# martin-velas/SLAM_plus_plus

Measured on AMD Instinct MI355X. Metric: Lambda solve GFLOP/s (algorithmic factor+solve flops / wall-clock), 100k-pose SE(3), higher is better.
Workload: dtype f64; 1 GPU; C3: synthetic 100000-pose SE(3) chain + loop closures, 6x6 blocks, 201998 upper blocks, n=600000; numeric factor + 2 substitutions per step (symbolic analysis cached, inputs resident in HBM); parallelism=1 GPU

## Files before the change

### slam_plus_plus_amd/csrc/panel_kernel.hip

```cpp
#include <hip/hip_runtime.h>
#include "sparse_kernels.h"

namespace slampp {

#include "sparse_device.inl"

template <int D, int BATCH>
__device__ __forceinline__ void panel_update_block(const TUpdSlot &sl, bool b_valid, const TUpdEnt *__restrict__ ents,
	const double *__restrict__ A, double *L, const double *__restrict__ b, double *w, int n_sub_wave, int n_waves, int lane,
	double *s_ops , double *s_yv , double *s_part )
{
	enum { DD = D * D };
	const TLaneMap mm = lane_map(lane, D, D);
	const bool b_diag = sl.kind != 0;
	const bool b_y = b_diag && lane >= Y_LANE0 && lane < Y_LANE0 + D;
	const int yq = b_y? lane - Y_LANE0 : mm.q;
	double init = 0;
	if(b_valid && n_sub_wave == 0)
		init = b_y? b[sl.cs_src + yq] : (mm.b_act? lambda_element(A, sl.asrc, mm.r, mm.q, D, D, false) : 0.0);
	double sum = 0;
	const TUpdEnt *p_ent = ents + sl.e0;
	const int ne = b_valid? sl.ne : 0;
	for(int e0 = n_sub_wave * BATCH; e0 < ne; e0 += n_waves * BATCH) {
		const int n_here = min(int(BATCH), ne - e0);
// ... 397 lines not shown
			const double init = b_y? s_w[ci * D + yq] : (mm.b_act? s_L[col.slot0 * DD + lane] : 0.0);
			double sum = 0;
			for(int e = 0; e < col.inr; ++ e) {
				const uint32_t en = s_irow[col.ir0 + e];
				sum += row_product_image<D>(s_L + int(en & 0xffff) * DD, s_w + int(en >> 16) * D, mm.r, yq, b_y);
			}
			TColDesc cd;
			cd.linv_off = col.linv_off;
			cd.cs_new = col.cs_new;
			const double acc = init - sum;
			finish_diagonal_fixed<D>(cd, acc, acc, lane, b_y? 0 : mm.r, b_y? 0 : mm.q, mm.b_act, L, Linv, w, s_slot[col.slot0].loff,
				p_flag, s_linv + (ci - ci0) * 64, s_L + col.slot0 * DD, s_w + ci * D);
		}
		__syncthreads();
		PANEL_TICK();
		int n_before = 0;
		for(int ci = ci0; ci < ci1; ++ ci) {
			const int n_slot0 = s_col[ci].slot0, n_nb = s_col[ci].nb;
			for(int kb = 1 + ((wave - n_before) % W + W) % W; kb < n_nb; kb += W) {
				const int n_slot = n_slot0 + kb;
				const TPanelSlot sd = s_slot[n_slot];
				const double init = mm.b_act? s_L[n_slot * DD + lane] : 0.0;
				double sum = 0;
				for(int e = 0; e < sd.inp; ++ e) {
					const uint32_t en = s_ipair[sd.ip0 + e];
					sum += pair_product_image<D>(s_L + int(en & 0xffff) * DD, s_L + int(en >> 16) * DD, mm.r, mm.q);
				}
				finish_offdiagonal<D>(init - sum, lane, mm.r, mm.q, mm.b_act, D, L, sd.loff, s_tile, s_linv + (ci - ci0) * 64, s_L + n_slot * DD);
			}
			n_before += n_nb - 1;
		}
		__syncthreads();
		PANEL_TICK();
		ci0 = ci1;
	}
	panel_hand_up<D>(s_out, n_out, 0, n_out, wave, W, lane, mm, b_y, yq, s_L, s_w, H);
	PANEL_TICK();
}

bool launch_factor_panel(int n_dim, bool b_fused, bool b_rows, const TPanelLaunch &r_cfg, const longlong2 *pkg, const int64_t *pkg_off, const int64_t *out_off,
	int n_tasks, const TUpdSlot *upd_slots, int n_upd_slots, const TUpdEnt *upd_ents, const double *A, const double *b, double *L, double *Linv, double *w,
	double *H, int *p_flag, hipStream_t stream, long long *p_timing, const TBatch &t_batch)
{
	if(!b_fused)
		n_upd_slots = 0;
	const int W = r_cfg.n_waves, n_groups = W / std::min(W, int(PANEL_UPD_W));
	const int n_grid = n_tasks + (n_upd_slots + n_groups - 1) / n_groups;
	if(n_grid <= 0)
		return true;
	const size_t n_lds_bytes = size_t(panel_lds(n_dim, b_fused, r_cfg).TOTAL) * sizeof(double);
	if(n_lds_bytes > PANEL_LDS_BUDGET)
		return false;
#define LAUNCH_PANEL_INSTANCE(D, WW, F, RW) do { \
		static bool b_attribute_set = false; \
		if(!b_attribute_set) { \
			(void)hipFuncSetAttribute(reinterpret_cast<const void*>(&factor_panel_kernel<D, WW, F, RW>), hipFuncAttributeMaxDynamicSharedMemorySize, 160 * 1024); \
			b_attribute_set = true; \
		} \
		hipLaunchKernelGGL((factor_panel_kernel<D, WW, F, RW>), dim3(n_grid, t_batch.n), dim3(64 * WW), n_lds_bytes, stream, pkg, pkg_off, out_off, n_tasks, r_cfg, \
			upd_slots, n_upd_slots, upd_ents, A, b, L, Linv, w, H, p_flag, p_timing, t_batch); } while(0)
#define LAUNCH_PANEL_F(D, WW, F) do { if(b_rows) LAUNCH_PANEL_INSTANCE(D, WW, F, true); else LAUNCH_PANEL_INSTANCE(D, WW, F, false); } while(0)
#define LAUNCH_PANEL(D) do { \
		if(W == 2) { if(b_fused) LAUNCH_PANEL_F(D, 2, true); else LAUNCH_PANEL_F(D, 2, false); } \
		else if(W == 4) { if(b_fused) LAUNCH_PANEL_F(D, 4, true); else LAUNCH_PANEL_F(D, 4, false); } \
		else { if(b_fused) LAUNCH_PANEL_F(D, 8, true); else LAUNCH_PANEL_F(D, 8, false); } } while(0)
	switch(n_dim) {
	case 3:
		LAUNCH_PANEL(3);
		return true;
	case 6:
		LAUNCH_PANEL(6);
		return true;
	case 7:
		LAUNCH_PANEL(7);
		return true;
	default:
		return false;
	}
#undef LAUNCH_PANEL
#undef LAUNCH_PANEL_F
#undef LAUNCH_PANEL_INSTANCE
}

template <int D>
__global__ void __launch_bounds__(64 * PANEL_UPD_W)
panel_update_kernel(const TUpdSlot *__restrict__ slots, const TUpdEnt *__restrict__ ents, const double *__restrict__ A, double *L,
	const double *__restrict__ b, double *w, TBatch t_batch)
{	{ const int64_t n_member = blockIdx.y; A += n_member * t_batch.a; L += n_member * t_batch.l; b += n_member * t_batch.b; w += n_member * t_batch.w; }

	enum { W = PANEL_UPD_W, DD = D * D, BATCH = 8 };
	__shared__ double s_ops[W][2 * BATCH * DD];
	__shared__ double s_yv[W][BATCH * 8];
	__shared__ double s_part[W][64];
	const int wave = threadIdx.x >> 6, lane = threadIdx.x & 63;
	const TUpdSlot sl = slots[blockIdx.x];
	panel_update_block<D, BATCH>(sl, true, ents, A, L, b, w, wave, W, lane, s_ops[wave], s_yv[wave], s_part[0]);
}

void launch_panel_update(int n_dim, const TUpdSlot *slots, int n_slots, const TUpdEnt *ents, const double *A, double *L,
	const double *b, double *w, hipStream_t stream, const TBatch &t_batch)
{
	if(n_slots <= 0)
		return;
	if(n_dim == 3)
		hipLaunchKernelGGL((panel_update_kernel<3>), dim3(n_slots, t_batch.n), dim3(64 * PANEL_UPD_W), 0, stream, slots, ents, A, L, b, w, t_batch);
	else if(n_dim == 6)
		hipLaunchKernelGGL((panel_update_kernel<6>), dim3(n_slots, t_batch.n), dim3(64 * PANEL_UPD_W), 0, stream, slots, ents, A, L, b, w, t_batch);
	else
		hipLaunchKernelGGL((panel_update_kernel<7>), dim3(n_slots, t_batch.n), dim3(64 * PANEL_UPD_W), 0, stream, slots, ents, A, L, b, w, t_batch);
}

}

#include "preload.h"
SLAMPP_PRELOAD_UNIT(panel_kernel)
```

### slam_plus_plus_amd/csrc/solver.h

```cpp
#pragma once
#include <hip/hip_runtime.h>
#include <chrono>
#include <cstdint>
#include <new>
#include <stdexcept>
#include <string>
#include <vector>
#include <thread>
#include <memory>
#include <mutex>

#include "../../include/slampp_hip.h"
#include "plan.h"
#include <utility>
#include "sparse_kernels.h"
#include "dense_chol.h"

namespace slampp {

struct CDeviceError : public std::runtime_error {
	explicit CDeviceError(const std::string &s) :std::runtime_error(s) {}
};

#define SLAMPP_HIP_CHECK(call) do { hipError_t e_ = (call); if(e_ != hipSuccess) { \
// ... 81 lines not shown
template <class T> using raw_vector = std::vector<T, CNoInitAlloc<T> >;

struct TTrash { virtual ~TTrash() {} };
template <class T> struct TTrashOf : TTrash { T t; explicit TTrashOf(T &r) { t.swap(r); } };
typedef std::vector<std::unique_ptr<TTrash> > CTrashList;
template <class T> inline void Discard_Later(CTrashList &r_trash, T &r_v) { r_trash.emplace_back(new TTrashOf<T>(r_v)); }

struct CKeepDeviceMemory {
	bool b_before;
	CKeepDeviceMemory() :b_before(g_b_keep_device_memory) { g_b_keep_device_memory = true; }
	~CKeepDeviceMemory() { g_b_keep_device_memory = b_before; }
};

struct CSchurState;
struct CDeviceGroup;
struct CSparseInverse;
struct CCovariance;
struct CAssemblyState;

}

struct slampp_hip_assembly {
	slampp_hip_solver *p_solver;
	slampp::CAssemblyState *p_state;
	bool b_stale;
};

struct slampp_hip_solver {
	int n_device;
	hipStream_t stream;
	std::string s_error;
	slampp::PlanOptions opt;
	int n_dense_nb;
	int b_shard_primary;
	int n_shard_rank, n_shard_world;
	int n_marginals_dense;
	int n_assembly_groups = 1 << 20;
	int n_schur_tiles = -1;
	int n_schur_incremental = 0;
	int n_schur_sparse;

	bool b_has_structure, b_analyzed, b_factored;
	uint64_t n_factor_gen = 0, n_schur_cov_gen = 0;
	int n_mode;
	int64_t n_matrix_cut;
	std::vector<int64_t> cumsum, bcol_ptr;
	std::vector<int32_t> brow;
	int64_t n_values, n_scalars;

	bool b_refined = false;
	int64_t n_refined_values = 0;
	std::vector<int64_t> refined_cumsum, refined_bcol_ptr;
	std::vector<int32_t> refined_brow;
	slampp::CDevArray<int64_t> d_refine_map;
	slampp::CDevArray<double> d_refined;
	void Refine_Structure();
	bool b_schur_fallback = false;
	int n_staging_ahead = 0;
	int n_schur_fallback_option = 1;
	slampp::Plan plan;
	int n_bottom_stages;
	slampp::TDevPlan dplan;
	slampp::CDevArray<slampp::TColDesc> d_cols;
	slampp::CDevArray<slampp::TBlkDesc> d_blks;
	slampp::CDevArray<slampp::TRowEnt> d_rents;
	slampp::CDevArray<longlong2> d_pairs;
	slampp::CDevArray<int64_t> d_task_ptr, d_task_pkg;
	slampp::CDevArray<longlong2> d_pkg;
	slampp::CDevArray<long long> d_timing;
	slampp::CDevArray<slampp::TSimtChunk> d_simt_chunks;
	slampp::CDevArray<int32_t> d_simt_prog, d_simt_rest;
	int n_panel = -1;
	int n_panel_rows = -1;
	slampp::CDevArray<longlong2> d_panel_pkg;
	slampp::CDevArray<int64_t> d_panel_off, d_panel_out_off;
	slampp::CDevArray<double> d_handup;
	bool b_any_hand_up = false;
	int n_panel_handup = 1;
	slampp::CDevArray<int32_t> d_panel_rest;
	slampp::CDevArray<slampp::TUpdSlot> d_panel_upd_slots;
	slampp::CDevArray<slampp::TUpdEnt> d_panel_upd_ents;
	std::vector<int32_t> panel_ptr, panel_rest_ptr, panel_upd_ptr;
	std::vector<slampp::TPanelLaunch> panel_cfg;
	std::vector<char> panel_ride;
	slampp::CDevArray<int64_t> d_simt_tab;
	slampp::CDevArray<slampp::TSimtChunk> d_simt_bwd_chunks;
	slampp::CDevArray<int32_t> d_simt_bwd_prog;
	slampp::CDevArray<int64_t> d_simt_bwd_tab;
	std::vector<int32_t> simt_bwd_lds_bytes;
	std::vector<slampp::TSimtChunk> simt_host_bwd_chunks;
	std::vector<int32_t> simt_host_bwd_prog;
	slampp::raw_vector<int64_t> simt_host_bwd_tab;
	bool b_leaf_linv_wanted = false, b_leaf_linv_valid = true;
	slampp::TBatch t_batch = slampp::t_No_Batch();
	slampp::CDevArray<double> d_batch_L, d_batch_Linv, d_batch_w, d_batch_handup;
	slampp::CDevArray<int> d_batch_flag;
	int n_batch_owner_member = -1;
	int *p_host_batch_flag = 0;
	int n_batch_pending = 0;
	int n_simt_backward = -1;
	void Ensure_Leaf_Inverses();
	std::vector<int32_t> simt_chunk_ptr, simt_rest_ptr;
	std::vector<int32_t> simt_lds_bytes;
	int n_simt = -1;
	int n_wide_min_tasks = 8192;
	int n_simt_width = 32;
	int n_simt_stages = 1;
	void Build_Simt();
	void Upload_Simt();
	std::vector<slampp::TSimtChunk> simt_host_chunks;
	std::vector<int32_t> simt_host_prog, simt_host_rest;
	slampp::raw_vector<int64_t> simt_host_tab;
	slampp::CDevArray<slampp::TDenseBlk> d_dense_blks;
	slampp::CDevArray<int64_t> d_dense_blk_loff;
	slampp::CDevArray<double> d_dense, d_dense_invdiag, d_dense_z, d_dense_x;
	slampp::CDevArray<int32_t> d_dense_gaps;
	int n_dense_gaps;
	slampp::CDevArray<uint8_t> d_dense_unit;
	slampp::CDevArray<longlong2> d_dense_dst;
	slampp::CTileSchedule dense_tiles;
	bool b_dense_tiles;
	bool b_dense_clean;
	int n_dense_top_tiles;
	int n_dense_blks, n_dense_cols, n_dense_dim, n_dense_pad;
	slampp::CDevArray<double> d_A, d_rhs, d_L, d_Linv, d_w, d_cov;
	slampp::CSparseInverse *p_sinv = 0;
	bool b_sinv_tried = false;
	slampp::CCovariance *p_cov = 0;
	slampp::CDevArray<double> d_Z;
	slampp::CDevArray<double> d_Zd, d_Zd_work;
	slampp::CDevArray<int64_t> d_diag_zoff;
	slampp::CDevArray<int32_t> d_diag_dim;
	slampp::CDevArray<int64_t> d_diag_out_off;
	slampp::CDevArray<int64_t> d_damp_off;
	bool b_damp_valid = false;
	slampp::CDevArray<int> d_flag;
	int *p_flag_shared = 0;
	int *p_host_flag;

	double *p_pin_values = 0, *p_pin_rhs = 0;
	size_t n_pin_values = 0, n_pin_rhs = 0;
	bool b_pin_values_registered = false, b_pin_rhs_registered = false;
	bool b_pin_values_deferred = false, b_pin_rhs_deferred = false;
	bool b_staging_ever = false;
	std::thread t_staging_registration;
	void Register_Staging_Later();
	void Join_Staging_Registration();
	slampp::CTrashList analysis_trash;
	std::thread t_discard;
	void Join_Discard() { if(t_discard.joinable()) t_discard.join(); }
	std::thread t_bringup;
	std::mutex m_bringup;
	int n_bringup_status = SLAMPP_HIP_OK;
	int n_Join_Bringup()
	{
		std::lock_guard<std::mutex> t_lock(m_bringup);
		if(t_bringup.joinable()) {
			const double t0 = slampp::wall_ms();
			t_bringup.join();
			if(getenv("SLAMPP_HIP_PLAN_TIMING"))
				fprintf(stderr, "[bring-up] waited for %.2f ms\n", slampp::wall_ms() - t0);
		}
		return n_bringup_status;
	}
	void Join_Bringup()
	{
// ... 96 lines not shown
```

### slam_plus_plus_amd/csrc/sparse_enqueue.hip

```cpp
#include <execinfo.h>
#include <signal.h>
#include <unistd.h>
#include <pthread.h>
#include "solver.h"
#include "sparse_inverse.h"

#include <algorithm>
#include <atomic>
#include <chrono>
#include <cstdio>
#include <cstdlib>
#include <cstring>
#include <map>
#include <thread>
#include <mutex>
#include <condition_variable>
#include <functional>
#include <sys/mman.h>

using namespace slampp;

void slampp_hip_solver::Enqueue_Sparse(const double *p_values_dev, double *p_rhs_dev, bool b_factor, bool b_factor_only)
{
	const Plan &P = plan;
// ... 60 lines not shown
				}
			} else if(s == 0 && !panel_ptr.empty() && panel_ptr[1] > panel_ptr[0]) {
				Launch_Panels(s, true);
			} else if(s > 0 && s < n_bottom_stages && dplan.task_pkg)
				launch_factor_wide(dplan, p_values_dev, d_L.p(), d_Linv.p(), p_rhs_dev, d_w.p(), P.stage_ptr[s],
					P.stage_ptr[s + 1] - P.stage_ptr[s], p_flag, stream, t_batch);
			else if(s >= n_bottom_stages && !panel_ptr.empty()) {
				Launch_Panels(s, false);
			} else
			launch_factor_stage(dplan, p_values_dev, d_L.p(), d_Linv.p(), p_rhs_dev, d_w.p(), P.stage_ptr[s],
				P.stage_ptr[s + 1] - P.stage_ptr[s], s < n_bottom_stages, p_flag, stream, t_batch);
			if(s == 0 || (s == n_wide_end - 1 && b_profile >= 2) || s == n_stages - 1)
				Phase_End();
		}
	} else {
		Phase_Begin("forward");
		for(int s = 0; s < n_stages; ++ s) {
			launch_forward_stage(dplan, d_L.p(), d_Linv.p(), p_rhs_dev, d_w.p(), P.stage_ptr[s],
				P.stage_ptr[s + 1] - P.stage_ptr[s], stream);
		}
		Phase_End();
	}
	if(b_factor_only && !n_dense_dim) {
		SLAMPP_HIP_CHECK(hipGetLastError());
		return;
	}
	if(n_dense_dim) {
		const int ld = n_dense_pad;
		if(b_factor) {
			Phase_Begin("dense_assemble");
			if(b_dense_tiles && b_dense_clean)
				tile_zero(dense_tiles, d_dense.p(), ld, stream, d_dense_unit.p());
			else {
				SLAMPP_HIP_CHECK(hipMemsetAsync(d_dense.p(), 0, size_t(ld) * ld * sizeof(double), stream));
				b_dense_clean = b_dense_tiles;
				dense_prepare_padding(d_dense.p(), ld, n_dense_dim, stream);
				dense_prepare_gaps(d_dense.p(), ld, d_dense_gaps.p(), n_dense_gaps, stream);
			}
			launch_dense_assemble(dplan, d_dense_blks.p(), n_dense_blks, p_values_dev, d_L.p(), p_rhs_dev, d_w.p(),
				d_dense.p(), ld, false, stream);
			Phase_End();
			Phase_Begin("dense_chol");
			if(b_dense_tiles)
				tile_cholesky(dense_tiles, d_dense.p(), ld, n_dense_dim, d_dense_invdiag.p(), p_flag, stream);
			else
				dense_cholesky(d_dense.p(), ld, n_dense_dim, d_dense_invdiag.p(), p_flag, stream);
			Phase_End();
			if(b_factor_only) {
				launch_dense_gather_factor(d_dense_blks.p(), d_dense_blk_loff.p(), n_dense_blks, d_dense.p(), ld, d_L.p(), stream);
				SLAMPP_HIP_CHECK(hipGetLastError());
				return;
			}
		} else {
			Phase_Begin("dense_forward");
			launch_dense_assemble(dplan, d_dense_blks.p(), n_dense_blks, 0, d_L.p(), p_rhs_dev, d_w.p(),
				d_dense.p(), ld, true, stream);
			dense_forwardsolve(d_dense.p(), ld, d_dense_invdiag.p(), stream);
			Phase_End();
		}
		Phase_Begin("dense_solve");
		if(b_dense_tiles)
			tile_backsolve(dense_tiles, d_dense.p(), ld, n_dense_dim, d_dense_invdiag.p(), d_dense_z.p(), d_dense_x.p(), stream,
				d_dense_dst.p(), d_w.p(), p_rhs_dev);
		else
		dense_backsolve(d_dense.p(), ld, n_dense_dim, d_dense_invdiag.p(), d_dense_z.p(), d_dense_x.p(), stream,
			d_dense_dst.p(), d_w.p(), p_rhs_dev);
		Phase_End();
	}
	Phase_Begin("backward");
	for(int s = n_stages; s > 0; -- s) {
		if(b_simt_bwd && s < int(simt_chunk_ptr.size())) {
			const int n_chunks = simt_chunk_ptr[s] - simt_chunk_ptr[s - 1], n_rest = simt_rest_ptr[s] - simt_rest_ptr[s - 1];
			launch_backward_simt(d_simt_bwd_chunks.p() + simt_chunk_ptr[s - 1], n_chunks, n_simt_width, simt_bwd_lds_bytes[s - 1],
				d_simt_bwd_prog.p(), d_simt_bwd_tab.p(), P.max_dim, d_L.p(), d_w.p(), p_rhs_dev, stream, t_batch);
			if(n_rest > 0) {
				TDevPlan t_rest = dplan;
				t_rest.task_map = d_simt_rest.p();
				launch_backward_stage(t_rest, d_L.p(), d_Linv.p(), d_w.p(), p_rhs_dev, simt_rest_ptr[s - 1], n_rest, stream, t_batch);
			}
			continue;
		}
		if(s < int(simt_chunk_ptr.size()))
			Ensure_Leaf_Inverses();
		launch_backward_stage(dplan, d_L.p(), d_Linv.p(), d_w.p(), p_rhs_dev, P.stage_ptr[s - 1],
			P.stage_ptr[s] - P.stage_ptr[s - 1], stream, t_batch);
	}
	Phase_End();
	SLAMPP_HIP_CHECK(hipGetLastError());
}
```

### slam_plus_plus_amd/csrc/sparse_kernels.h

```cpp
#pragma once
#include <hip/hip_runtime.h>
#include <stdint.h>
#include "plan.h"

namespace slampp {

struct TBatch {
	int n;
	int64_t a, l, linv, b, w, h;
};
inline TBatch t_No_Batch() { TBatch t = {1, 0, 0, 0, 0, 0, 0}; return t; }



struct TColDesc {
	int64_t k0;
	int32_t nb, dj;
	int64_t linv_off;
	int64_t cs_new;
	int64_t cs_src;
	int64_t r0;
	int32_t nr;
	int32_t np;
	int64_t p0;
};

struct TBlkDesc {
	int64_t loff;
	int64_t asrc;
	int64_t p0;
	uint32_t np_di;
	int32_t xcs;
};

struct TRowEnt {
	int64_t off;
	int32_t ycs;
	int32_t dc;
};

struct TDenseBlk {
	int64_t asrc;
	int64_t p0;
	int64_t dst;
	int64_t r0;
	int32_t np, nr;
	int32_t di, dj;
	int64_t cs_src;
	int32_t pos;
	int32_t pad;
};

struct TDenseCol {
	int64_t cs_new, cs_src;
	int32_t pos, dj;
};

enum { PANEL_W = 8, PANEL_COLS = 8, PANEL_UNITS = 1024, PANEL_UPD_W = 4 };
struct TPanelHead {
	int32_t n_cols, n_slots, n_units, n_int_rows;
	int32_t ext_ptr[12];
};
struct TPanelOut {
	int32_t op0, onp;
	int64_t dst;
};
struct TPanelCol {
	int64_t linv_off, cs_new, cs_src;
	int32_t slot0, nb;
	int32_t ir0, inr;
	int32_t sub, pad;
};
struct TPanelSlot {
	int64_t loff, asrc;
	int32_t ip0, inp;
	int64_t pad;
};
struct TPanelExt {
	int64_t a_off, b_off;
	int32_t ycs;
	uint16_t slot, kind;
	int32_t col;
	int32_t pad;
};
struct TUpdSlot {
	int64_t loff, asrc;
	int64_t e0;
	int32_t ne, kind;
	int64_t cs_src, cs_new;
	int64_t pad[2];
};
struct TUpdEnt {
	int64_t a_off;
	int64_t b_off;
};
inline int panel_slot_cap(int n_dim) { return (n_dim == 6)? 96 : (n_dim == 7)? 72 : 256; }

struct TPanelLaunch {
	int32_t n_waves, n_cap_units, n_cap_blk, n_cap_cols, n_cap_lvl;
	int32_t n_cap_out;
	int32_t b_from_lambda;
};
enum { PANEL_UPD_BATCH = 8 };
inline __host__ __device__ constexpr int panel_fresh_batch(int n_waves) { return (n_waves == 4)? 8 : 4; }
struct TPanelLds {
	int IMAGE, VEC, LINV, TILE, OPS, YV, OUT, TOTAL;
};
enum { PANEL_LDS_BUDGET = 156 * 1024 };
inline __host__ __device__ TPanelLds panel_lds(int D, bool b_fused, const TPanelLaunch &c)
{
	const int DD = D * D, W = c.n_waves;
	TPanelLds l;
	l.IMAGE = 2 * c.n_cap_units;
	l.VEC = l.IMAGE + c.n_cap_blk * DD;
	l.LINV = l.VEC + c.n_cap_cols * 8;
	l.TILE = l.LINV + c.n_cap_cols * 64;
	l.OPS = l.TILE + W * 64;
	l.YV = l.OPS + (b_fused? W * 2 * panel_fresh_batch(W) * DD : 0);
	l.OUT = l.YV + (b_fused? W * panel_fresh_batch(W) * 8 : 0);
	const int n_panel_end = l.OUT + 2 * c.n_cap_out;
	const int n_upd_end = b_fused? W * 2 * PANEL_UPD_BATCH * DD + W * PANEL_UPD_BATCH * 8 + W * 64 : 0;
	l.TOTAL = (n_panel_end > n_upd_end)? n_panel_end : n_upd_end;
	return l;
}

bool launch_factor_panel(int n_dim, bool b_fused, bool b_rows, const TPanelLaunch &r_cfg, const longlong2 *pkg, const int64_t *pkg_off, const int64_t *out_off,
	int n_tasks, const TUpdSlot *upd_slots, int n_upd_slots, const TUpdEnt *upd_ents, const double *A, const double *b, double *L, double *Linv, double *w,
	double *H, int *p_flag, hipStream_t stream, long long *p_timing = 0, const TBatch &t_batch = t_No_Batch());
void launch_panel_update(int n_dim, const TUpdSlot *slots, int n_slots, const TUpdEnt *ents, const double *A, double *L,
	const double *b, double *w, hipStream_t stream, const TBatch &t_batch = t_No_Batch());

enum { UP_CHUNK = 16, UP_NR = 128, UP_NP = 512, WIDE_CHUNK = 8, WIDE_NR = 32, WIDE_NP = 48 };
enum { PKG_SPECULATIVE = 512 };

inline __host__ __device__ int package_units(int nb, int ne)
{
	return 4 + 2 * nb + ne + (ne + 3) / 4 + (ne + 15) / 16;
}

struct TDevPlan {
	const TColDesc *cols;
	const TBlkDesc *blks;
	const longlong2 *pairs;
	const TRowEnt *rents;
	const int64_t *task_ptr;
	int uniform_dim;
	int64_t n_blks, n_pairs, n_rents;
	const longlong2 *pkg;
	const int64_t *task_pkg;
	const int32_t *task_map;
	long long *p_timing;
};

struct TSimtChunk {
	int32_t prog_off;
	int32_t n_tasks;
	int64_t tab_off;
};

bool launch_factor_simt(const TSimtChunk *chunks, int n_chunks, int n_width ,
	int n_lds_bytes ,
	const int32_t *prog, const int64_t *tab, int n_dim,
	const double *A, double *L, double *Linv , const double *b, double *w, int *p_flag, hipStream_t stream,
	long long *p_timing = 0 , const TBatch &t_batch = t_No_Batch());
bool launch_backward_simt(const TSimtChunk *chunks, int n_chunks, int n_width, int n_lds_bytes, const int32_t *prog, const int64_t *tab,
	int n_dim, const double *L, double *w, double *x_out, hipStream_t stream, const TBatch &t_batch = t_No_Batch());
bool launch_invert_diagonals(const TDevPlan &p, int64_t col_begin, int64_t col_end, const double *L, double *Linv, hipStream_t stream);

void launch_factor_stage(const TDevPlan &p, const double *A, double *L, double *Linv, const double *b,
	double *w, int task_begin, int n_tasks, bool b_bottom_stage, int *p_flag, hipStream_t stream, const TBatch &t_batch = t_No_Batch());
bool launch_factor_subtree_image(const TDevPlan &p, const double *A, double *L, double *Linv, const double *b,
	double *w, int task_begin, int n_tasks, int *p_flag, hipStream_t stream, const TBatch &t_batch = t_No_Batch());
void launch_factor_wide(const TDevPlan &p, const double *A, double *L, double *Linv, const double *b,
	double *w, int task_begin, int n_tasks, int *p_flag, hipStream_t stream, const TBatch &t_batch = t_No_Batch());
void launch_forward_stage(const TDevPlan &p, const double *L, const double *Linv, const double *b,
	double *w, int task_begin, int n_tasks, hipStream_t stream);
void launch_backward_stage(const TDevPlan &p, const double *L, const double *Linv, double *w,
	double *x_out, int task_begin, int n_tasks, hipStream_t stream, const TBatch &t_batch = t_No_Batch());

void launch_dense_assemble(const TDevPlan &p, const TDenseBlk *blks, int n_blks, const double *A, const double *L,
	const double *b, const double *w, double *Dm, int ld, bool b_rhs_only, hipStream_t stream);
void launch_dense_gather_factor(const TDenseBlk *blks, const int64_t *loffs, int n_blks, const double *Dm, int ld, double *L, hipStream_t stream);
void launch_gather_values(const int64_t *p_map, int64_t n, const double *p_src, double *p_dst, hipStream_t stream);

}
```

### slam_plus_plus_amd/csrc/sparse_setup.hip

```cpp
#include <execinfo.h>
#include <signal.h>
#include <unistd.h>
#include <pthread.h>
#include "solver.h"
#include "sparse_inverse.h"

#include <algorithm>
#include <atomic>
#include <chrono>
#include <cstdio>
#include <cstdlib>
#include <cstring>
#include <map>
#include <unordered_map>
#include <thread>
#include <mutex>
#include <condition_variable>
#include <functional>
#include <sys/mman.h>

using namespace slampp;

void slampp_hip_solver::Refine_Structure()
{
// ... 380 lines not shown
				if(!b_fits) {
					if(n_slots <= n_slot_cap && n_cols >= 1 && n_cols <= int(PANEL_COLS))
						Release_Slots();
					panel_rest.push_back(t);
					continue;
				}
				irow.clear(); ipair.clear(); pcols.clear(); pslots.clear(); fresh.clear();
				for(size_t o = 0; o < order.size(); ++ o)
					col_local[P.task_cols[order[o]]] = int32_t(o);
				auto Hand_Up = [&](int64_t ka, int64_t kb, int64_t n_target, int32_t n_col_here, int32_t n_slot_here, bool b_diag) {
					const int32_t n_src = col_package[P.blk_col[ka]];
					const std::pair<int32_t, int64_t> key(n_src, n_target);
					std::map<std::pair<int32_t, int64_t>, int32_t>::iterator it = out_of.find(key);
					THandUp &r_up = hand_up[size_t(n_src)];
					if(it == out_of.end()) {
						TPanelOut rec;
						rec.op0 = -1;
						rec.onp = 0;
						rec.dst = n_handup_doubles | (int64_t(b_diag) << 62);
						it = out_of.insert(std::make_pair(key, int32_t(r_up.recs.size()))).first;
						r_up.recs.push_back(rec);
						TPanelExt en;
						memset(&en, 0, sizeof(en));
						en.a_off = n_handup_doubles;
						en.slot = uint16_t(n_slot_here);
						en.kind = b_diag? 3 : 2;
						en.col = n_col_here;
						fresh.push_back(en);
						n_handup_doubles += P.max_dim * P.max_dim + 8;
					}
					r_up.recs[size_t(it->second)].onp = std::max(r_up.recs[size_t(it->second)].onp, col_level[P.blk_col[ka]]);
					r_up.pairs.push_back(uint32_t(it->second));
					r_up.pairs.push_back(b_diag? (uint32_t(img_slot[ka]) | (uint32_t(col_local[P.blk_col[ka]]) << 16)) :
						(uint32_t(img_slot[ka]) | (uint32_t(img_slot[kb]) << 16)));
				};
				for(size_t o = 0; o < order.size(); ++ o) {
					const int64_t i = order[o];
					const TColDesc &c = cols[i];
					TPanelCol pc;
					memset(&pc, 0, sizeof(pc));
					pc.linv_off = c.linv_off;
					pc.cs_new = c.cs_new;
					pc.cs_src = c.cs_src;
					pc.slot0 = slot_of[c.k0];
					pc.nb = c.nb;
					pc.sub = b_tall? P.col_sub[P.task_cols[i]] : int32_t(o);
					pc.ir0 = int32_t(irow.size());
					TUpdSlot us;
					memset(&us, 0, sizeof(us));
					us.loff = blks[c.k0].loff;
					us.asrc = blks[c.k0].asrc;
					us.e0 = int64_t(upd_ents.size());
					us.kind = 1;
					us.cs_src = c.cs_src;
					us.cs_new = c.cs_new;
					for(int64_t e = c.r0; e < c.r0 + c.nr; ++ e) {
						const int64_t k = P.rblk[e];
						if(slot_of[k] >= 0)
							irow.push_back(uint32_t(slot_of[k]) | (uint32_t(col_local[P.blk_col[k]]) << 16));
						else if(Handed_Up(k))
							Hand_Up(k, k, c.k0, int32_t(o), pc.slot0, true);
						else if(b_ride && (b_self || col_stage[P.blk_col[k]] == s - 1)) {
							TPanelExt en;
							memset(&en, 0, sizeof(en));
							en.a_off = en.b_off = rents[e].off;
							en.ycs = rents[e].ycs;
							en.slot = uint16_t(pc.slot0);
							en.kind = 1;
							en.col = int32_t(o);
							fresh.push_back(en);
						} else
							upd_ents.push_back(TUpdEnt{rents[e].off, int64_t(rents[e].ycs)});
					}
					us.ne = int32_t(int64_t(upd_ents.size()) - us.e0);
					upd_slots.push_back(us);
					pc.inr = int32_t(irow.size()) - pc.ir0;
					pcols.push_back(pc);
					for(int64_t k = c.k0; k < c.k0 + c.nb; ++ k) {
						TPanelSlot ps;
						memset(&ps, 0, sizeof(ps));
						ps.loff = blks[k].loff;
						ps.asrc = blks[k].asrc;
						ps.ip0 = int32_t(ipair.size());
						if(k > c.k0) {
							memset(&us, 0, sizeof(us));
							us.loff = blks[k].loff;
							us.asrc = blks[k].asrc;
							us.e0 = int64_t(upd_ents.size());
							for(int64_t e = P.pptr[k]; e < P.pptr[k + 1]; ++ e) {
								const int64_t ka = P.pa[e], kb = P.pb[e];
								if(slot_of[ka] >= 0)
									ipair.push_back(uint32_t(slot_of[ka]) | (uint32_t(slot_of[kb]) << 16));
								else if(Handed_Up(ka))
									Hand_Up(ka, kb, k, 0, slot_of[k], false);
								else if(b_ride && (b_self || col_stage[P.blk_col[ka]] == s - 1)) {
									TPanelExt en;
									memset(&en, 0, sizeof(en));
									en.a_off = P.loff[ka];
									en.b_off = P.loff[kb];
									en.slot = uint16_t(slot_of[k]);
									fresh.push_back(en);
								} else
									upd_ents.push_back(TUpdEnt{P.loff[ka], P.loff[kb]});
							}
							us.ne = int32_t(int64_t(upd_ents.size()) - us.e0);
							upd_slots.push_back(us);
						}
						ps.inp = int32_t(ipair.size()) - ps.ip0;
						pslots.push_back(ps);
					}
				}
				TPanelHead hd;
				memset(&hd, 0, sizeof(hd));
				hd.n_cols = n_cols;
				hd.n_slots = int32_t(n_slots);
				hd.n_units = int32_t(n_units);
				hd.n_int_rows = int32_t(irow.size());
				std::stable_sort(fresh.begin(), fresh.end(), [n_stage_waves](const TPanelExt &x, const TPanelExt &y) {
					const int wx = x.slot % n_stage_waves, wy = y.slot % n_stage_waves, ux = x.kind < 2, uy = y.kind < 2;
					return wx < wy || (wx == wy && (ux < uy || (ux == uy && x.slot < y.slot))); });
				for(size_t e = 0; e < fresh.size(); ++ e)
					++ hd.ext_ptr[fresh[e].slot % n_stage_waves + 1];
				for(int v = 0; v < n_stage_waves; ++ v)
					hd.ext_ptr[v + 1] += hd.ext_ptr[v];
				{
					TPanelLaunch &r_cfg = panel_cfg[s];
					r_cfg.n_cap_units = std::max(r_cfg.n_cap_units, int32_t(n_units));
					r_cfg.n_cap_blk = std::max(r_cfg.n_cap_blk, int32_t(n_slots));
					r_cfg.n_cap_cols = std::max(r_cfg.n_cap_cols, int32_t(n_cols));
					int n_level_cols = 0, n_level = -1;
					for(size_t o = 0; o < pcols.size(); ++ o) {
						n_level_cols = (pcols[o].sub == n_level)? n_level_cols + 1 : 1;
						n_level = pcols[o].sub;
						r_cfg.n_cap_lvl = std::max(r_cfg.n_cap_lvl, int32_t(n_level_cols));
					}
				}
				if(int64_t(fresh.size()) != n_fresh)
					throw std::logic_error("panel package: fresh entries miscounted");
				const size_t n_at = panel_pkg.size();
				panel_pkg.resize(n_at + n_units, longlong2{0, 0});
				char *p_dst = reinterpret_cast<char*>(&panel_pkg[n_at]);
				memcpy(p_dst, &hd, sizeof(hd));
				p_dst += 64;
				memcpy(p_dst, pcols.data(), pcols.size() * sizeof(TPanelCol));
				p_dst += pcols.size() * sizeof(TPanelCol);
				memcpy(p_dst, pslots.data(), pslots.size() * sizeof(TPanelSlot));
				p_dst += pslots.size() * sizeof(TPanelSlot);
				if(!irow.empty())
					memcpy(p_dst, irow.data(), irow.size() * sizeof(uint32_t));
				p_dst += (irow.size() + 3) / 4 * 16;
				if(!ipair.empty())
					memcpy(p_dst, ipair.data(), ipair.size() * sizeof(uint32_t));
				p_dst += (ipair.size() + 3) / 4 * 16;
				if(!fresh.empty())
					memcpy(p_dst, fresh.data(), fresh.size() * sizeof(TPanelExt));
				for(size_t o = 0, n_level = 0; o < order.size(); ++ o) {
					const TColDesc &c = cols[order[o]];
					for(int64_t k = c.k0; k < c.k0 + c.nb; ++ k)
						img_slot[k] = slot_of[k];
					col_package[P.task_cols[order[o]]] = int32_t(panel_off.size());
					if(o > 0 && pcols[o].sub != pcols[o - 1].sub)
						++ n_level;
					col_level[P.task_cols[order[o]]] = int32_t(n_level);
				}
				panel_off.push_back(int64_t(n_at));
				panel_out_off.push_back(-1);
// ... 198 lines not shown
				const int32_t i = P.lrow[k];
				if(P.dense_pos[i] < 0)
					throw std::logic_error("dense top is not closed upwards");
				TDenseBlk b;
				memset(&b, 0, sizeof(b));
				b.asrc = (P.asrc[k] < 0)? -1 : P.asrc[k] * 2 + P.atrans[k];
				b.p0 = P.pptr[k];
				b.np = int32_t(P.pptr[k + 1] - P.pptr[k]);
				b.dst = int64_t(P.dense_pos[i]) + int64_t(P.dense_pos[j]) * n_dense_pad;
				b.di = P.dim[i]; b.dj = P.dim[j];
				if(k == P.lptr[j]) {
					b.r0 = P.rptr[j];
					b.nr = int32_t(P.rptr[j + 1] - P.rptr[j]);
					b.cs_src = P.cs_src[j];
					b.pos = P.dense_pos[j];
				} else
					b.nr = -1;
				dense_blks.push_back(b);
				dense_blk_loff.push_back(P.loff[k]);
			}
		}
		SETUP_PHASE("dense records");
		d_dense_blks.Upload(dense_blks, stream);
		d_dense_blk_loff.Upload(dense_blk_loff, stream);
		SETUP_PHASE("dense upload 1");
		{
			std::vector<char> covered(n_dense_dim, 0);
			for(size_t k = 0; k < dense_cols.size(); ++ k)
				std::fill(covered.begin() + dense_cols[k].pos, covered.begin() + dense_cols[k].pos + dense_cols[k].dj, char(1));
			std::vector<int32_t> gaps;
			for(int32_t q = 0; q < n_dense_dim; ++ q) {
				if(!covered[q])
					gaps.push_back(q);
			}
			n_dense_gaps = int(gaps.size());
			d_dense_gaps.Upload(gaps, stream);
			std::vector<uint8_t> unit(n_dense_pad, uint8_t(1));
			std::vector<longlong2> dst(n_dense_pad, longlong2{-1, -1});
			for(size_t k = 0; k < dense_cols.size(); ++ k) {
				for(int q = 0; q < dense_cols[k].dj; ++ q) {
					unit[dense_cols[k].pos + q] = 0;
					dst[dense_cols[k].pos + q] = longlong2{(long long)(dense_cols[k].cs_new + q), (long long)(dense_cols[k].cs_src + q)};
				}
			}
			d_dense_unit.Upload(unit, stream);
			d_dense_dst.Upload(dst, stream);
			SETUP_PHASE("dense upload 2");
			SLAMPP_HIP_CHECK(hipStreamSynchronize(stream));
		}
		SETUP_PHASE("dense lists");
		d_dense.Alloc(size_t(n_dense_pad) * n_dense_pad);
		b_dense_clean = false;
		d_dense_invdiag.Alloc(size_t(n_dense_pad / dense_NB) * dense_NB * dense_NB);
		d_dense_z.Alloc(n_dense_pad);
		d_dense_x.Alloc(n_dense_pad);
		SETUP_PHASE("dense allocs");
		b_dense_tiles = false;
		if(n_dense_top_tiles != 0) {
			std::vector<char> nonzero;
			const int T = dense_top_tile_pattern(P, nonzero);
			if(T != n_dense_pad / dense_NB)
				throw std::logic_error("dense top: tile count mismatch");
			if(dense_tiles.Build(T, nonzero, stream))
				b_dense_tiles = n_dense_top_tiles > 0 || 100 * dense_tiles.n_levels <= 85 * T;
			if(b_timing) {
				size_t n_nz = 0;
				for(size_t k = 0; k < nonzero.size(); ++ k)
					n_nz += nonzero[k];
				fprintf(stderr, "[setup] dense top: %d tiles per side, %zu of %d lower tiles nonzero before fill, %d levels, "
					"%d trsm tiles, %d update targets -> %s schedule\n", T, n_nz, T * (T + 1) / 2, dense_tiles.n_levels,
					dense_tiles.level_trsm_ptr.empty()? 0 : dense_tiles.level_trsm_ptr.back(),
					dense_tiles.level_tgt_ptr.empty()? 0 : dense_tiles.level_tgt_ptr.back(), b_dense_tiles? "tile" : "dense");
			}
		}
	}
	n_dense_blks = int(dense_blks.size());
	n_dense_cols = int(dense_cols.size());
	SETUP_PHASE("tile schedule");
	if(t_panel_thread.t.joinable())
		t_panel_thread.t.join();
	if(p_panel_error)
		std::rethrow_exception(p_panel_error);
	SETUP_PHASE("packages");
	d_panel_upd_slots.Upload(upd_slots, stream);
	d_panel_upd_ents.Upload(upd_ents, stream);
	d_panel_pkg.Upload(panel_pkg, stream);
	d_panel_off.Upload(panel_off, stream);
	d_panel_out_off.Upload(panel_out_off, stream);
	d_handup.Alloc(size_t(std::max<int64_t>(n_handup_doubles, int64_t(P.max_dim) * P.max_dim + 8)));
	d_panel_rest.Upload(panel_rest, stream);
	if(t_upload_thread.t.joinable())
		t_upload_thread.t.join();
	if(p_upload_error)
		std::rethrow_exception(p_upload_error);
	SETUP_PHASE("uploads");
	d_L.Alloc(size_t(P.loff[n_lblocks]));
	d_Linv.Alloc(size_t(P.linv_off[P.n]));
	d_w.Alloc(size_t(P.cs_new[P.n]));
	d_flag.Alloc(1);
	SLAMPP_HIP_CHECK(hipMemsetAsync(d_flag.p(), 0, sizeof(int), stream));
	SETUP_PHASE("allocs");
	SLAMPP_HIP_CHECK(hipStreamSynchronize(stream));
	SETUP_PHASE("sync");
#undef SETUP_PHASE

	dplan.cols = d_cols.p(); dplan.blks = d_blks.p(); dplan.pairs = d_pairs.p(); dplan.rents = d_rents.p();
	dplan.task_ptr = d_task_ptr.p();
	dplan.uniform_dim = P.uniform_dim? P.max_dim : 0;
	dplan.pkg = d_pkg.p();
	dplan.task_pkg = d_pkg.p()? d_task_pkg.p() : 0;
	dplan.n_blks = n_lblocks;
	dplan.n_pairs = int64_t(pairs.size());
	dplan.n_rents = int64_t(rents.size());
	dplan.p_timing = 0;
	dplan.task_map = 0;
	{
		const double t_wait = wall_ms();
		if(t_simt_thread.t.joinable())
			t_simt_thread.t.join();
		if(p_simt_error)
			std::rethrow_exception(p_simt_error);
		Upload_Simt();
		if(b_timing)
			fprintf(stderr, "[setup] %-12s %8.2f ms since it was started, %.2f ms of them waited for\n", "shapes", wall_ms() - t_simt, wall_ms() - t_wait);
	}
	if(getenv("SLAMPP_HIP_STAGE_TIMING")) {
		d_timing.Alloc(1 + 32 * 4096);
		SLAMPP_HIP_CHECK(hipMemsetAsync(d_timing.p(), 0, (1 + 32 * 4096) * sizeof(long long), stream));
		dplan.p_timing = d_timing.p();
	}
	if(!b_small) {
		Join_Discard();
		Discard_Later(analysis_trash, cols); Discard_Later(analysis_trash, blks); Discard_Later(analysis_trash, pairs);
		Discard_Later(analysis_trash, rents); Discard_Later(analysis_trash, pkg); Discard_Later(analysis_trash, task_pkg);
		Discard_Later(analysis_trash, panel_pkg); Discard_Later(analysis_trash, upd_slots); Discard_Later(analysis_trash, upd_ents);
		try {
			t_discard = std::thread([this]() { analysis_trash.clear(); host_pool_release(); });
		} catch(std::system_error&) {
			analysis_trash.clear();
			host_pool_release();
		}
	}
}

void slampp_hip_solver::Build_Simt()
{
	simt_chunk_ptr.clear();
	simt_rest_ptr.clear();
	simt_lds_bytes.clear();
	simt_host_chunks.clear(); simt_host_prog.clear(); simt_host_tab.clear(); simt_host_rest.clear();
	simt_bwd_lds_bytes.clear();
	simt_host_bwd_chunks.clear(); simt_host_bwd_prog.clear(); simt_host_bwd_tab.clear();
	const Plan &P = plan;
	if(!n_simt || !P.uniform_dim || (P.max_dim != 3 && P.max_dim != 6 && P.max_dim != 7))
		return;
	if(n_simt < 0 && P.stage_ptr.size() > 1 && P.stage_ptr[1] - P.stage_ptr[0] < 2048)
		return;
	enum { MIN_GROUP = 1, MAX_PROG = 4096, MAX_TABLE_BYTES = 40960 };
	const int n_stages = int(P.stage_ptr.size()) - 1;
	std::vector<TSimtChunk> &chunks = simt_host_chunks;
	std::vector<int32_t> &prog_all = simt_host_prog, &rest = simt_host_rest;
	raw_vector<int64_t> &tab = simt_host_tab;
	size_t n_tab_size = 0, n_bwd_tab_size = 0;
	struct TTask { int32_t n_task; bool b_fits; uint64_t n_hash; std::vector<int32_t> prog, ops, ys; };
	simt_chunk_ptr.push_back(0);
	simt_rest_ptr.push_back(0);
// ... 277 lines not shown
```

Measured before the change: 521.0 GFLOP/s.

## Add panel-based backward substitution kernel reusing factor panel packages

Adds a backward-substitution kernel that works on the same panel packages used by the panel factorization. It stages each panel's L/Linv blocks and rhs vectors into LDS, then solves the panel's columns level by level inside one workgroup, with wave-level shuffles doing the reductions. Leftover tasks go through the existing backward stage. The aim is fewer per-stage backward launches and less global traffic in the substitution, at the cost of LDS capacity limits and extra slot tags encoded into the packages during setup.

```diff
diff --git a/slam_plus_plus_amd/csrc/panel_kernel.hip b/slam_plus_plus_amd/csrc/panel_kernel.hip
--- a/slam_plus_plus_amd/csrc/panel_kernel.hip
+++ b/slam_plus_plus_amd/csrc/panel_kernel.hip
@@ -503,6 +503,127 @@
 #undef LAUNCH_PANEL_INSTANCE
 }
 
+template <int D, int W, int U>
+__global__ void __launch_bounds__(64 * W)
+backward_panel_kernel(const longlong2 *__restrict__ pkg, const int64_t *__restrict__ pkg_off, int n_cap_units, int n_cap_blk,
+	const double *__restrict__ L, const double *__restrict__ Linv, double *w, double *__restrict__ x_out, TBatch t_batch)
+{	{ const int64_t n_member = blockIdx.y; L += n_member * t_batch.l; Linv += n_member * t_batch.linv; w += n_member * t_batch.w; x_out += n_member * t_batch.b; }
+
+	enum { DD = D * D };
+	static_assert(DD + D <= 64, "a slot's block and its vector share a wave's lanes");
+	extern __shared__ __attribute__((aligned(16))) double s_raw[];
+	longlong2 *s_pkg = reinterpret_cast<longlong2*>(s_raw);
+	double *s_L = s_raw + 2 * n_cap_units, *s_x = s_L + n_cap_blk * DD, *s_xi = s_x + n_cap_blk * 8;
+	const int tid = threadIdx.x, wave = tid >> 6, lane = tid & 63;
+	const int64_t n_off = pkg_off[blockIdx.x];
+	s_pkg[tid] = pkg[n_off + tid];
+	__syncthreads();
+	const TPanelHead *p_hd = reinterpret_cast<const TPanelHead*>(s_pkg);
+	const int n_cols = p_hd->n_cols, n_slots = p_hd->n_slots;
+	const int n_need = 4 + 3 * n_cols + 2 * n_slots;
+	if(n_need > 64 * W) {
+		for(int e = 64 * W + tid; e < n_need; e += 64 * W)
+			s_pkg[e] = pkg[n_off + e];
+		__syncthreads();
+	}
+	const TPanelCol *s_col = reinterpret_cast<const TPanelCol*>(s_pkg + 4);
+	const TPanelSlot *s_slot = reinterpret_cast<const TPanelSlot*>(s_pkg + 4 + 3 * n_cols);
+
+	const bool b_el = lane < DD, b_vec = lane >= DD && lane < DD + D;
+	for(int s0 = wave; s0 < n_slots; s0 += U * W) {
+		double v[U];
+		#pragma unroll
+		for(int u = 0; u < U; ++ u) {
+			const int n_slot = min(s0 + u * W, n_slots - 1);
+			const int64_t n_tag = s_slot[n_slot].pad;
+			const int64_t n_blk = ((n_tag >> 48) & 1)? s_col[int(n_tag >> 40) & 0xff].linv_off : s_slot[n_slot].loff;
+			const double *p_blk = (((n_tag >> 48) & 1)? Linv : L) + n_blk + (b_el? lane : 0);
+			const double *p_src = b_vec? w + int64_t(uint32_t(n_tag)) + (lane - DD) : p_blk;
+			v[u] = *p_src;
+		}
+		#pragma unroll
+		for(int u = 0; u < U; ++ u) {
+			const int n_slot = s0 + u * W;
+			if(n_slot < n_slots) {
+				if(b_el)
+					s_L[n_slot * DD + lane] = v[u];
+				else if(b_vec)
+					s_x[n_slot * 8 + (lane - DD)] = v[u];
+			}
+		}
+	}
+	__syncthreads();
+
+	const int g = lane >> 3, q = lane & 7, qq = (q < D)? q : 0;
+	for(int ci1 = n_cols; ci1 > 0;) {
+		const int n_sub = s_col[ci1 - 1].sub;
+		int ci0 = ci1 - 1;
+		while(ci0 > 0 && s_col[ci0 - 1].sub == n_sub)
+			-- ci0;
+		for(int ci = ci0 + wave; ci < ci1; ci += W) {
+			const int n_slot0 = s_col[ci].slot0, n_nb = s_col[ci].nb;
+			double acc = 0;
+			for(int kb = 1 + g; kb < n_nb; kb += 8) {
+				const int n_slot = n_slot0 + kb;
+				const int n_row_col = int(s_slot[n_slot].pad >> 32) & 0xff;
+				const double *p_x = (n_row_col != int(PANEL_ROW_OUTSIDE))? s_xi + n_row_col * 8 : s_x + n_slot * 8;
+				const double *p_l = s_L + n_slot * DD + qq * D;
+				#pragma unroll
+				for(int t = 0; t < D; ++ t)
+					acc += p_l[t] * p_x[t];
+			}
+			acc += __shfl_xor(acc, 8);
+			acc += __shfl_xor(acc, 16);
+			acc += __shfl_xor(acc, 32);
+			const double val = (q < D)? s_x[n_slot0 * 8 + qq] - acc : 0;
+			const double *p_li = s_L + n_slot0 * DD + qq * D;
+			double x = 0;
+			#pragma unroll
+			for(int t = 0; t < D; ++ t) {
+				const double vt = __shfl(val, t);
+				if(t >= qq)
+					x += p_li[t] * vt;
+			}
+			if(lane < D) {
+				s_xi[ci * 8 + lane] = x;
+				w[s_col[ci].cs_new + lane] = x;
+				x_out[s_col[ci].cs_src + lane] = x;
+			}
+		}
+		if(ci0 > 0)
+			__syncthreads();
+		ci1 = ci0;
+	}
+}
+
+bool launch_backward_panel(int n_dim, int n_waves, const TPanelLaunch &r_cfg, const longlong2 *pkg, const int64_t *pkg_off, int n_tasks,
+	const double *L, const double *Linv, double *w, double *x_out, hipStream_t stream, const TBatch &t_batch)
+{
+	if(n_dim != 3 && n_dim != 6 && n_dim != 7)
+		return false;
+	if(n_tasks <= 0)
+		return true;
+	const int W = (n_waves <= 2)? 2 : 4;
+	const int n_cap_units = std::max(64 * W, 4 + 3 * r_cfg.n_cap_cols + 2 * r_cfg.n_cap_blk);
+	const size_t n_lds_bytes = (size_t(2) * n_cap_units + size_t(r_cfg.n_cap_blk) * (n_dim * n_dim + 8) + size_t(r_cfg.n_cap_cols) * 8) * sizeof(double);
+	if(n_lds_bytes > 64 * 1024)
+		return false;
+#define LAUNCH_BACKWARD_PANEL_W(D, WW, UU) hipLaunchKernelGGL((backward_panel_kernel<D, WW, UU>), dim3(n_tasks, t_batch.n), dim3(64 * WW), n_lds_bytes, stream, \
+		pkg, pkg_off, n_cap_units, r_cfg.n_cap_blk, L, Linv, w, x_out, t_batch)
+#define LAUNCH_BACKWARD_PANEL(D) do { \
+		if(W == 2) LAUNCH_BACKWARD_PANEL_W(D, 2, 8); \
+		else LAUNCH_BACKWARD_PANEL_W(D, 4, 8); } while(0)
+	if(n_dim == 3)
+		LAUNCH_BACKWARD_PANEL(3);
+	else if(n_dim == 6)
+		LAUNCH_BACKWARD_PANEL(6);
+	else
+		LAUNCH_BACKWARD_PANEL(7);
+#undef LAUNCH_BACKWARD_PANEL_W
+#undef LAUNCH_BACKWARD_PANEL
+	return true;
+}
+
 template <int D>
 __global__ void __launch_bounds__(64 * PANEL_UPD_W)
 panel_update_kernel(const TUpdSlot *__restrict__ slots, const TUpdEnt *__restrict__ ents, const double *__restrict__ A, double *L,
diff --git a/slam_plus_plus_amd/csrc/solver.h b/slam_plus_plus_amd/csrc/solver.h
--- a/slam_plus_plus_amd/csrc/solver.h
+++ b/slam_plus_plus_amd/csrc/solver.h
@@ -187,6 +187,7 @@
 	slampp::CDevArray<slampp::TUpdEnt> d_panel_upd_ents;
 	std::vector<int32_t> panel_ptr, panel_rest_ptr, panel_upd_ptr;
 	std::vector<slampp::TPanelLaunch> panel_cfg;
+	std::vector<int32_t> panel_bwd_waves;
 	std::vector<char> panel_ride;
 	slampp::CDevArray<int64_t> d_simt_tab;
 	slampp::CDevArray<slampp::TSimtChunk> d_simt_bwd_chunks;
diff --git a/slam_plus_plus_amd/csrc/sparse_enqueue.hip b/slam_plus_plus_amd/csrc/sparse_enqueue.hip
--- a/slam_plus_plus_amd/csrc/sparse_enqueue.hip
+++ b/slam_plus_plus_amd/csrc/sparse_enqueue.hip
@@ -166,6 +166,17 @@
 		}
 		if(s < int(simt_chunk_ptr.size()))
 			Ensure_Leaf_Inverses();
+		else if(s <= int(panel_bwd_waves.size()) && panel_bwd_waves[s - 1] > 0 &&
+		   launch_backward_panel(P.max_dim, panel_bwd_waves[s - 1], panel_cfg[s - 1], d_panel_pkg.p(), d_panel_off.p() + panel_ptr[s - 1],
+		   panel_ptr[s] - panel_ptr[s - 1], d_L.p(), d_Linv.p(), d_w.p(), p_rhs_dev, stream, t_batch)) {
+			if(panel_rest_ptr[s] > panel_rest_ptr[s - 1]) {
+				TDevPlan t_rest = dplan;
+				t_rest.task_map = d_panel_rest.p();
+				launch_backward_stage(t_rest, d_L.p(), d_Linv.p(), d_w.p(), p_rhs_dev, panel_rest_ptr[s - 1],
+					panel_rest_ptr[s] - panel_rest_ptr[s - 1], stream, t_batch);
+			}
+			continue;
+		}
 		launch_backward_stage(dplan, d_L.p(), d_Linv.p(), d_w.p(), p_rhs_dev, P.stage_ptr[s - 1],
 			P.stage_ptr[s] - P.stage_ptr[s - 1], stream, t_batch);
 	}
diff --git a/slam_plus_plus_amd/csrc/sparse_kernels.h b/slam_plus_plus_amd/csrc/sparse_kernels.h
--- a/slam_plus_plus_amd/csrc/sparse_kernels.h
+++ b/slam_plus_plus_amd/csrc/sparse_kernels.h
@@ -76,6 +76,11 @@
 	int32_t ip0, inp;
 	int64_t pad;
 };
+enum { PANEL_ROW_OUTSIDE = 0xff };
+inline __host__ __device__ int64_t panel_slot_tag(int32_t n_xcs, int32_t n_row_col, int32_t n_col, bool b_diag)
+{
+	return int64_t(uint32_t(n_xcs)) | (int64_t(n_row_col & 0xff) << 32) | (int64_t(n_col & 0xff) << 40) | (int64_t(b_diag) << 48);
+}
 struct TPanelExt {
 	int64_t a_off, b_off;
 	int32_t ycs;
@@ -127,6 +132,8 @@
 bool launch_factor_panel(int n_dim, bool b_fused, bool b_rows, const TPanelLaunch &r_cfg, const longlong2 *pkg, const int64_t *pkg_off, const int64_t *out_off,
 	int n_tasks, const TUpdSlot *upd_slots, int n_upd_slots, const TUpdEnt *upd_ents, const double *A, const double *b, double *L, double *Linv, double *w,
 	double *H, int *p_flag, hipStream_t stream, long long *p_timing = 0, const TBatch &t_batch = t_No_Batch());
+bool launch_backward_panel(int n_dim, int n_waves, const TPanelLaunch &r_cfg, const longlong2 *pkg, const int64_t *pkg_off, int n_tasks,
+	const double *L, const double *Linv, double *w, double *x_out, hipStream_t stream, const TBatch &t_batch = t_No_Batch());
 void launch_panel_update(int n_dim, const TUpdSlot *slots, int n_slots, const TUpdEnt *ents, const double *A, double *L,
 	const double *b, double *w, hipStream_t stream, const TBatch &t_batch = t_No_Batch());
 
diff --git a/slam_plus_plus_amd/csrc/sparse_setup.hip b/slam_plus_plus_amd/csrc/sparse_setup.hip
--- a/slam_plus_plus_amd/csrc/sparse_setup.hip
+++ b/slam_plus_plus_amd/csrc/sparse_setup.hip
@@ -486,6 +486,11 @@
 						ps.loff = blks[k].loff;
 						ps.asrc = blks[k].asrc;
 						ps.ip0 = int32_t(ipair.size());
+						{
+							const int32_t n_row = P.lrow[k];
+							const bool b_row_here = k > c.k0 && slot_of[P.lptr[n_row]] >= 0;
+							ps.pad = panel_slot_tag(int32_t(P.cs_new[n_row]), b_row_here? col_local[n_row] : int32_t(PANEL_ROW_OUTSIDE), int32_t(o), k == c.k0);
+						}
 						if(k > c.k0) {
 							memset(&us, 0, sizeof(us));
 							us.loff = blks[k].loff;
@@ -850,6 +855,15 @@
 	if(p_panel_error)
 		std::rethrow_exception(p_panel_error);
 	SETUP_PHASE("packages");
+	panel_bwd_waves.assign(panel_ptr.empty()? size_t(0) : panel_ptr.size() - 1, 0);
+	if(!dev_knob_set("SLAMPP_HIP_DEV_BACKWARD_STAGE")) {
+		const int n_bwd_w2_min_tasks = dev_knob("SLAMPP_HIP_DEV_BACKWARD_W2_MIN", 1024);
+		const int n_bwd_waves = dev_knob("SLAMPP_HIP_DEV_BACKWARD_W", 4), n_bwd_waves_crowded = dev_knob("SLAMPP_HIP_DEV_BACKWARD_W_CROWDED", 2);
+		for(size_t s = 0; s < panel_bwd_waves.size(); ++ s) {
+			if(panel_ptr[s + 1] > panel_ptr[s])
+				panel_bwd_waves[s] = (panel_ptr[s + 1] - panel_ptr[s] > n_bwd_w2_min_tasks)? n_bwd_waves_crowded : n_bwd_waves;
+		}
+	}
 	d_panel_upd_slots.Upload(upd_slots, stream);
 	d_panel_upd_ents.Upload(upd_ents, stream);
 	d_panel_pkg.Upload(panel_pkg, stream);
```

After: 524.2 GFLOP/s (median of 6 runs). About the same (+0.6%).
